# tonyjohnvan/ACE-Step-1.5

Hardware: AMD Instinct MI355X
Metric: seconds/song (240 s audio, 27 DiT steps) (lower is better)
Workload: dtype bf16

## Files before the change

### ace-step-1.5_amd/csrc/gemm.hip

```cpp
#include <hip/hip_ext.h>

#include "kernels.h"
#include "headpost.h"

namespace acehip {
namespace {

constexpr int BK = 64;
constexpr int GROUP_M = 8;

#ifdef GEMM_STAMPS
constexpr int STAMP_WG = 16384;
__device__ unsigned long long g_gemm_stamps[STAMP_WG * 2 * 8];
__device__ __forceinline__ void stamp(int slot, int i, unsigned long long v) {
    if (slot < STAMP_WG * 2) {
        asm volatile("" : "+v"(v));
        g_gemm_stamps[slot * 8 + i] = v;
    }
}
#define GSTAMP(i)                                                                                \
    do {                                                                                         \
        if ((threadIdx.x & 255) == 0 && threadIdx.x < 512) stamp(blockIdx.x * 2 + (threadIdx.x >> 8), i, __builtin_amdgcn_s_memtime()); \
    } while (0)
#define GSTAMP_REAL(i)                                                                           \
    do {                                                                                         \
        if ((threadIdx.x & 255) == 0 && threadIdx.x < 512) stamp(blockIdx.x * 2 + (threadIdx.x >> 8), i, __builtin_amdgcn_s_memrealtime()); \
    } while (0)
#else
#define GSTAMP(i) do {} while (0)
#define GSTAMP_REAL(i) do {} while (0)
#endif

struct ExtEvents {
    hipEvent_t start = nullptr, stop = nullptr;
};
thread_local ExtEvents g_ext_ev;
template <typename... KArgs, typename... Args>
inline void klaunch(void (*kern)(KArgs...), dim3 grid, dim3 block, hipStream_t s, Args... args) {
    if (g_ext_ev.stop) {
        hipEvent_t st = g_ext_ev.start;
        g_ext_ev.start = nullptr;
        hipExtLaunchKernelGGL(kern, grid, block, 0, s, st, g_ext_ev.stop, 0, args...);
    } else {
        kern<<<grid, block, 0, s>>>(args...);
    }
}
__device__ __forceinline__ int swz(int row, int chunk) { return row * 128 + ((chunk ^ ((row >> 1) & 7)) << 4); }

template <int N>
__device__ __forceinline__ void ring_barrier() {
    asm volatile("s_waitcnt vmcnt(%0) lgkmcnt(0)" ::"n"(N) : "memory");
    __builtin_amdgcn_s_barrier();
    asm volatile("" ::: "memory");
}

template <int SM, int SN, int EPI, int CHMAX = 12>
__device__ __forceinline__ void epilogue_tile(const GemmArgs &a, const f32x4 (&acc)[SM][SN], int row0, int col0,
                                              int fr, int fc) {
    static_assert(SN % 2 == 0, "sub-tiles are paired");
    const bool odd = fc & 1;
    const int cpos = (fc >> 1) * 8;
#pragma unroll
    for (int i = 0; i < SM; ++i) {
        const int m = row0 + i * 16 + fr;
        const bool live = m < a.M;
        if constexpr (EPI == EPI_SWIGLU) {
#pragma unroll
            for (int pnl = 0; pnl < SN / 4; ++pnl) {
                f32x4 p0, p1;
                float o[8];
                float g8[8], u8[8];
#pragma unroll
                for (int r = 0; r < 4; ++r) {
                    g8[r] = acc[i][4 * pnl][r];
                    g8[4 + r] = acc[i][4 * pnl + 1][r];
                    u8[r] = acc[i][4 * pnl + 2][r];
                    u8[4 + r] = acc[i][4 * pnl + 3][r];
                }
                rbf_n<8>(g8);
                rbf_n<8>(u8);
#pragma unroll
                for (int r = 0; r < 8; ++r) g8[r] = silu_f(g8[r]);
                rbf_n<8>(g8);
#pragma unroll
                for (int r = 0; r < 4; ++r) {
                    p0[r] = g8[r] * u8[r];
                    p1[r] = g8[4 + r] * u8[4 + r];
                }
                pair8(p0, p1, odd, o);
                const int nout = ((col0 + pnl * 64) >> 1) + (odd ? 16 : 0) + cpos;
                if (live) *(uint4 *)(a.C + (int64_t)m * a.ldc + nout) = pack8(o);
            }
        }
    }
    if constexpr (EPI == EPI_CONV) {
        constexpr int NP = SN / 2;
        uint4 bz[NP];
        float sav[NP][8], sbv[NP][8];
        int colv[NP], phv[NP];
#pragma unroll
        for (int jp = 0; jp < NP; ++jp) {
            const int n = col0 + (2 * jp + (odd ? 1 : 0)) * 16 + cpos;
            phv[jp] = n / a.conv_cout;
            colv[jp] = n - phv[jp] * a.conv_cout;
            bz[jp] = a.bias ? *(const uint4 *)(a.bias + colv[jp]) : make_uint4(0, 0, 0, 0);
            if (a.Cs) {
                const float4 a0 = *(const float4 *)(a.sa + colv[jp]), a1 = *(const float4 *)(a.sa + colv[jp] + 4);
                const float4 b0 = *(const float4 *)(a.sib + colv[jp]), b1 = *(const float4 *)(a.sib + colv[jp] + 4);
                sav[jp][0] = a0.x; sav[jp][1] = a0.y; sav[jp][2] = a0.z; sav[jp][3] = a0.w;
                sav[jp][4] = a1.x; sav[jp][5] = a1.y; sav[jp][6] = a1.z; sav[jp][7] = a1.w;
                sbv[jp][0] = b0.x; sbv[jp][1] = b0.y; sbv[jp][2] = b0.z; sbv[jp][3] = b0.w;
                sbv[jp][4] = b1.x; sbv[jp][5] = b1.y; sbv[jp][6] = b1.z; sbv[jp][7] = b1.w;
            }
        }
// ... 274 lines not shown
        const int r = r0 + RPI * it;
        float x[8], cs[8] = {}, sn[8] = {};
        unpack8(*(const uint4 *)(st + r * PITCH + hh * 128 + d), x);
        if constexpr (MODE >= 2) {
            unpack8(cv[it], cs);
            unpack8(sv[it], sn);
        }
        if constexpr (MODE == 1) head_norm_rope_t<true, false>(x, li, w, cs, sn, h.eps);
        else if constexpr (MODE == 2) head_norm_rope_t<true, true>(x, li, w, cs, sn, h.eps);
        else if constexpr (MODE == 3) head_norm_rope(x, li, norm, w, h.cos != nullptr, cs, sn, h.eps);
        if (m0 + r < a.M) *(uint4 *)(base + (int64_t)bq * bstride + sq * 128) = pack8(x);
        sq += RPI;
        while (sq >= h.S) { sq -= h.S; ++bq; }
    }
}

template <int BM, int NW, int LDS_BYTES, int HPT, typename StoreAcc>
__device__ __forceinline__ void headpost_epilogue(const GemmArgs &a, char *lds, int m0, int n0, int wave, int lane,
                                                  StoreAcc store_acc) {
    static_assert(HPT == 1 || HPT == 2, "one or two heads per tile");
    constexpr int PITCH = 128 * HPT + 8;
    constexpr int RPW = 4 / HPT;
    constexpr int RPI = RPW * NW;
    constexpr int ITER = BM / RPI;
    static_assert(BM % RPI == 0, "rows must split evenly over the iterations");
    static_assert(BM * PITCH * 2 <= LDS_BYTES, "head-post staging tile must fit the operand ring");
    const HeadPostArgs &h = a.hp;
    const int sub = lane >> 4, li = lane & 15, d = li * 8, hh = HPT == 2 ? sub & 1 : 0;
    const int head = (n0 >> 7) + hh;
    const int nqk = h.nq + h.nk;
    const bool norm = head < nqk;
    const bool rope = h.cos != nullptr;
    const int r0 = wave * RPW + (HPT == 2 ? sub >> 1 : sub);
    const int mf = min(m0 + r0, a.M - 1) + h.m_off;
    const int b0 = mf / h.S, s0 = mf - b0 * h.S;
    uint4 cv[ITER], sv[ITER];
    if (rope) {
        int sq = s0;
#pragma unroll
        for (int it = 0; it < ITER; ++it) {
            const int sc = min(sq, h.S - 1);
            cv[it] = *(const uint4 *)(h.cos + (int64_t)sc * 128 + d);
            sv[it] = *(const uint4 *)(h.sin + (int64_t)sc * 128 + d);
            sq += RPI;
            while (sq >= h.S) sq -= h.S;
        }
    }
    bf16_t *base;
    int64_t bstride;
    const int64_t hs = (int64_t)h.S_dst * 128;
    if (head < h.nq) {
        const int64_t hq = h.S_dst_q ? (int64_t)h.S_dst_q * 128 : hs;
        base = h.q + head * hq;
        bstride = h.nq * hq;
    } else if (head < nqk) {
        base = h.k + (head - h.nq) * hs;
        bstride = h.nk * hs;
    } else {
        base = h.v + (head - nqk) * hs;
        bstride = h.nv * hs;
    }
    base += d;
    float w[8] = {};
    if (norm) unpack8(*(const uint4 *)((head < h.nq ? h.qw : h.kw) + d), w);
    bf16_t *st = (bf16_t *)lds;
    __syncthreads();
    store_acc(st, PITCH);
    __syncthreads();
    const bool uniform = HPT == 1 || (h.nq % 2 == 0 && nqk % 2 == 0);
    if (uniform) {
        if ((n0 >> 7) >= nqk)
            headpost_rows<0, ITER, RPI, PITCH>(a, st, m0, r0, hh, li, d, b0, s0, base, bstride, norm, w, cv, sv);
        else if (!rope)
            headpost_rows<1, ITER, RPI, PITCH>(a, st, m0, r0, hh, li, d, b0, s0, base, bstride, norm, w, cv, sv);
        else
            headpost_rows<2, ITER, RPI, PITCH>(a, st, m0, r0, hh, li, d, b0, s0, base, bstride, norm, w, cv, sv);
    } else {
        headpost_rows<3, ITER, RPI, PITCH>(a, st, m0, r0, hh, li, d, b0, s0, base, bstride, norm, w, cv, sv);
    }
}

template <int BM>
constexpr int pp_lds_bytes() { return 2 * (BM + 256) * 128; }
template <int BM, int EPI>
__device__ __forceinline__ void gemm_pp_body(const GemmArgs &a, char *lds, int bid) {
    constexpr int BN = 256, TM = BM / 2, SM = TM / 16, SMH = SM / 2;
    constexpr int ROWS = BM + BN, BUF = ROWS * 128;
    constexpr int NA = BM / 64, NB = BN / 64;
    static_assert(SM % 2 == 0, "A half must be whole 16-row sub-tiles");

    GSTAMP(0);
    GSTAMP_REAL(4);
    const int tid = threadIdx.x, lane = tid & 63, wave = tid >> 6;
    const int wr = wave >> 2, wc = wave & 3;
    const int tilesM = (a.M + BM - 1) / BM, tilesN = a.N / BN;
    const int nwg = tilesM * tilesN;
    const int wg = xcd_remap(bid, nwg);
    const int per_group = GROUP_M * tilesN;
    const int gid = wg / per_group, first_m = gid * GROUP_M;
    const int gsz = min(tilesM - first_m, GROUP_M);
    const int tm = first_m + (wg % per_group) % gsz;
    const int tn = (wg % per_group) / gsz;
    const int m0 = tm * BM, n0 = tn * BN;
#ifdef GEMM_STAMPS
    {
        unsigned xcc;
        asm volatile("s_getreg_b32 %0, hwreg(HW_REG_XCC_ID)" : "=s"(xcc));
        if ((threadIdx.x & 255) == 0) stamp(blockIdx.x * 2 + (threadIdx.x >> 8), 6, ((unsigned long long)wg << 32) | xcc);
    }
#endif

    const bf16_t *srcA[NA], *srcB[NB];
#pragma unroll
    for (int i = 0; i < NA; ++i) {
        const int r = (wave + 8 * i) * 8 + (lane >> 3);
        const int c = (lane & 7) ^ ((r >> 1) & 7);
        srcA[i] = a.A + (int64_t)min(m0 + r, a.M - 1) * a.lda + c * 8;
    }
#pragma unroll
    for (int i = 0; i < NB; ++i) {
        const int r = (wave + 8 * i) * 8 + (lane >> 3);
        const int c = (lane & 7) ^ (((BM + r) >> 1) & 7);
        srcB[i] = a.W + (int64_t)(n0 + r) * a.ldw + c * 8;
    }
    auto stageA = [&](int buf, int k0) {
        char *b = lds + buf * BUF;
        int ko = k0;
        if constexpr (EPI == EPI_CONV) {
            const int cin = a.conv_cin, tap = k0 / cin;
            ko = k0 + tap * (a.conv_dil - 1) * cin + a.conv_a0 * cin;
        }
#pragma unroll
        for (int i = 0; i < NA; ++i) glds16(srcA[i] + ko, b + (wave + 8 * i) * 1024);
    };
    auto stageB = [&](int buf, int k0) {
        char *b = lds + buf * BUF + BM * 128;
#pragma unroll
        for (int i = 0; i < NB; ++i) glds16(srcB[i] + k0, b + (wave + 8 * i) * 1024);
    };
    auto bar = [] {
        __builtin_amdgcn_sched_barrier(0);
        __builtin_amdgcn_s_barrier();
        __builtin_amdgcn_sched_barrier(0);
    };

    f32x4 acc[SM][4];
#pragma unroll
    for (int i = 0; i < SM; ++i)
#pragma unroll
        for (int j = 0; j < 4; ++j) acc[i][j] = f32x4{0.f, 0.f, 0.f, 0.f};

    const int fr = lane & 15, fc = lane >> 4;
    const int arow = wr * TM, brow = BM + wc * 64;

    const int nk = a.K / BK;
    stageB(0, 0);
    stageA(0, 0);
    if (nk > 1) {
        stageB(1, BK);
        asm volatile("s_waitcnt vmcnt(%0)" ::"n"(NB) : "memory");
    } else {
        asm volatile("s_waitcnt vmcnt(0)" ::: "memory");
    }
    bar();
    if (wr == 1) bar();
    GSTAMP(1);

    {
    bf16x8 xa[SMH][2], bf[4][2];
    auto readA = [&](const char *b, int h) {
#pragma unroll
        for (int i = 0; i < SMH; ++i)
#pragma unroll
            for (int ks = 0; ks < 2; ++ks)
                xa[i][ks] = *(const bf16x8 *)(b + swz(arow + (h * SMH + i) * 16 + fr, ks * 4 + fc));
    };
    auto mma = [&](int h) {
        __builtin_amdgcn_sched_barrier(0);
        __builtin_amdgcn_s_setprio(1);
#pragma unroll
        for (int ks = 0; ks < 2; ++ks)
#pragma unroll
            for (int i = 0; i < SMH; ++i)
#pragma unroll
                for (int j = 0; j < 4; ++j)
                    acc[h * SMH + i][j] = __builtin_amdgcn_mfma_f32_16x16x32_bf16(bf[j][ks], xa[i][ks], acc[h * SMH + i][j], 0, 0, 0);
        __builtin_amdgcn_s_setprio(0);
    };
    for (int kt = 0; kt < nk; ++kt) {
        const char *b = lds + (kt & 1) * BUF;
#pragma unroll
        for (int j = 0; j < 4; ++j)
#pragma unroll
            for (int ks = 0; ks < 2; ++ks) bf[j][ks] = *(const bf16x8 *)(b + swz(brow + j * 16 + fr, ks * 4 + fc));
        readA(b, 0);
        if (kt + 1 < nk) stageA((kt + 1) & 1, (kt + 1) * BK);
        asm volatile("s_waitcnt lgkmcnt(0)" ::: "memory");
        bar();
        mma(0);
        bar();
        readA(b, 1);
        if (kt + 2 < nk) {
            stageB(kt & 1, (kt + 2) * BK);
            asm volatile("s_waitcnt vmcnt(%0) lgkmcnt(0)" ::"n"(NB) : "memory");
        } else {
            asm volatile("s_waitcnt vmcnt(0) lgkmcnt(0)" ::: "memory");
        }
        bar();
        mma(1);
        bar();
    }
    }
    if (wr == 0) bar();
    GSTAMP(2);

    if constexpr (EPI == EPI_HEADPOST && BM == 256) {
#pragma unroll
        for (int hf = 0; hf < 2; ++hf)
            headpost_epilogue<128, 8, 2 * BUF, 2>(a, lds, m0 + hf * 128, n0, wave, lane, [&](bf16_t *st, int pitch) {
                if (wr != hf) return;
#pragma unroll
                for (int i = 0; i < SM; ++i)
#pragma unroll
                    for (int j = 0; j < 4; ++j) {
                        float o[4] = {acc[i][j][0], acc[i][j][1], acc[i][j][2], acc[i][j][3]};
                        *(uint2 *)(st + (i * 16 + fr) * pitch + wc * 64 + j * 16 + fc * 4) = pack4(o);
                    }
            });
        return;
    } else if constexpr (EPI == EPI_HEADPOST) {
        headpost_epilogue<BM, 8, 2 * BUF, 2>(a, lds, m0, n0, wave, lane, [&](bf16_t *st, int pitch) {
#pragma unroll
            for (int i = 0; i < SM; ++i)
#pragma unroll
                for (int j = 0; j < 4; ++j) {
                    float o[4] = {acc[i][j][0], acc[i][j][1], acc[i][j][2], acc[i][j][3]};
                    *(uint2 *)(st + (arow + i * 16 + fr) * pitch + wc * 64 + j * 16 + fc * 4) = pack4(o);
                }
        });
        return;
    }

    epilogue_tile<SM, 4, EPI>(a, acc, m0 + arow, n0 + wc * 64, fr, fc);
#ifdef GEMM_STAMPS
    asm volatile("s_waitcnt vmcnt(0)" ::: "memory");
#endif
    GSTAMP(3);
    GSTAMP_REAL(5);
}

template <int BM, int EPI>
__global__ __launch_bounds__(512, 1) void gemm_pp_kernel(GemmArgs a) {
    __shared__ __attribute__((aligned(16))) char lds[pp_lds_bytes<BM>()];
    gemm_pp_body<BM, EPI>(a, lds, blockIdx.x);
}

template <int EPI>
__global__ __launch_bounds__(512, 1) void gemm_pp_split_kernel(GemmArgs a, GemmArgs t, int nmain) {
    __shared__ __attribute__((aligned(16))) char lds[pp_lds_bytes<256>()];
    if ((int)blockIdx.x < nmain) gemm_pp_body<256, EPI>(a, lds, blockIdx.x);
    else gemm_pp_body<128, EPI>(t, lds, blockIdx.x - nmain);
}

template <int BM, int BN, int EPI, int NH = 0>
__global__ __launch_bounds__(256 + 64 * NH, 1) void gemm_w4_kernel(GemmArgs a) {
    constexpr int TM = BM / 2, TN = BN / 2, SM = TM / 16, SN = TN / 16;
    constexpr int ROWS = BM + BN, STAGE = ROWS * 128;
    constexpr int NS = 3 * STAGE <= 160 * 1024 ? 3 : 2;
    constexpr int PW = ROWS / 32;
    static_assert(ROWS % 32 == 0, "staging must split evenly over 4 waves");
    __shared__ __attribute__((aligned(16))) char lds[NS * STAGE];

    GSTAMP(0);
    GSTAMP_REAL(4);
    const int tid = threadIdx.x, lane = tid & 63, wave = tid >> 6;
    const int wm = wave >> 1, wn = wave & 1;
    const int tilesM = (a.M + BM - 1) / BM, tilesN = a.N / BN;
    const int nwg = tilesM * tilesN;
    const int wg = xcd_remap(blockIdx.x, nwg);
    const int per_group = GROUP_M * tilesN;
    const int gid = wg / per_group, first_m = gid * GROUP_M;
    const int gsz = min(tilesM - first_m, GROUP_M);
    const int tm = first_m + (wg % per_group) % gsz;
    const int tn = (wg % per_group) / gsz;
    const int m0 = tm * BM, n0 = tn * BN;
    const int nk = a.K / BK;

    if constexpr (NH > 0) {
        if (__builtin_amdgcn_readfirstlane(wave) >= 4) {
            constexpr int PPH = 4 * PW / NH;
            static_assert((4 * PW) % NH == 0 && (NS - 1) * PPH < 64, "helper pieces / vmcnt field");
            const int h = wave - 4;
            const bf16_t *hs[PPH];
#pragma unroll
            for (int i = 0; i < PPH; ++i) {
                const int q = h + NH * i, r = q * 8 + (lane >> 3);
                const int c = (lane & 7) ^ ((r >> 1) & 7);
                if (r < BM) hs[i] = a.A + (int64_t)min(m0 + r, a.M - 1) * a.lda + c * 8;
                else hs[i] = a.W + (int64_t)(n0 + r - BM) * a.ldw + c * 8;
            }
            auto fill = [&](int buf, int k0) {
#pragma unroll
                for (int i = 0; i < PPH; ++i) glds16(hs[i] + k0, lds + buf * STAGE + (h + NH * i) * 1024);
            };
            for (int t = 0; t < NS; ++t) fill(t, min(t, nk - 1) * BK);
            asm volatile("s_waitcnt vmcnt(%0)" ::"n"((NS - 1) * PPH) : "memory");
            __builtin_amdgcn_s_barrier();
            for (int kt = 0; kt < nk; ++kt) {
                asm volatile("s_waitcnt vmcnt(%0)" ::"n"((NS - 2) * PPH) : "memory");
                __builtin_amdgcn_s_barrier();
                asm volatile("" ::: "memory");
                fill(kt % NS, min(kt + NS, nk - 1) * BK);
            }
            asm volatile("s_waitcnt vmcnt(0)" ::: "memory");
            if constexpr (EPI == EPI_HEADPOST) {
                __syncthreads();
                __syncthreads();
            }
            return;
        }
    }

    const bf16_t *src[PW];
#pragma unroll
    for (int i = 0; i < PW; ++i) {
        const int r = (wave + 4 * i) * 8 + (lane >> 3);
        const int c = (lane & 7) ^ ((r >> 1) & 7);
        if (r < BM) src[i] = a.A + (int64_t)min(m0 + r, a.M - 1) * a.lda + c * 8;
        else src[i] = a.W + (int64_t)(n0 + r - BM) * a.ldw + c * 8;
    }
    auto stage1 = [&](int buf, int k0, int i) { glds16(src[i] + k0, lds + buf * STAGE + (wave + 4 * i) * 1024); };
// ... 116 lines not shown
        case EPI_SWIGLU: klaunch(gemm_pp_kernel<BM, EPI_SWIGLU>, dim3(tiles), dim3(512), s, a); break;
        case EPI_CONV:
            if constexpr (BM == 256 || BM == 128) {
                gemm_pp_kernel<BM, EPI_CONV><<<tiles, 512, 0, s>>>(a);
                break;
            }
            return fail(-1, "gemm: the conv epilogue runs on the 256- or 128-row ping-pong tile");
        case EPI_HEADPOST:
            if constexpr (BM == 256 || BM == 192 || BM == 128) {
                gemm_pp_kernel<BM, EPI_HEADPOST><<<tiles, 512, 0, s>>>(a);
                break;
            }
            return fail(-1, "gemm: head-post epilogue needs the 256-, 192- or 128-row ping-pong tile");
        default: return fail(-1, "gemm: bad epilogue");
    }
    HIP_TRY(hipGetLastError());
    return 0;
}

template <int BM, int BN, int WM, int WN, int STAGES, int NH = 0>
int launch(const GemmArgs &a, hipStream_t s) {
    if (a.N % BN) return fail(-1, "gemm: N not a multiple of the tile");
    const int tiles = ((a.M + BM - 1) / BM) * (a.N / BN);
    constexpr int NT = WM * WN * 64 + 64 * NH;
    switch (a.epi) {
        case EPI_STORE: gemm_kernel<BM, BN, WM, WN, STAGES, EPI_STORE, NH><<<tiles, NT, 0, s>>>(a); break;
        case EPI_GATED_RES: gemm_kernel<BM, BN, WM, WN, STAGES, EPI_GATED_RES, NH><<<tiles, NT, 0, s>>>(a); break;
        case EPI_RES: gemm_kernel<BM, BN, WM, WN, STAGES, EPI_RES, NH><<<tiles, NT, 0, s>>>(a); break;
        case EPI_SWIGLU: klaunch(gemm_kernel<BM, BN, WM, WN, STAGES, EPI_SWIGLU, NH>, dim3(tiles), dim3(NT), s, a); break;
        default: return fail(-1, "gemm: bad epilogue for this variant");
    }
    HIP_TRY(hipGetLastError());
    return 0;
}

}

int gemm_variant(const GemmArgs &a, int variant, hipStream_t s) {
    switch (variant) {
        case 0: return launch<128, 128, 2, 2, 2>(a, s);
        case 7: return launch_pp<256>(a, s);
        case 8: return launch_pp<192>(a, s);
        case 9: return launch_pp<128>(a, s);
        case 13: return knobs().gemm_helpers ? launch_w4<192, 128, 2>(a, s) : launch_w4<192, 128>(a, s);
        case 16: return launch<128, 64, 4, 1, 4>(a, s);
        case 17: return launch<128, 64, 4, 1, 4, 2>(a, s);
        default: return fail(-1, "gemm: bad variant (0, 7, 8, 9, 13, 16, 17)");
    }
}

#ifdef GEMM_STAMPS
}
extern "C" int acehip_diag_gemm_stamps(void *host, int n_wg) {
    n_wg = std::min(n_wg, acehip::STAMP_WG);
    HIP_TRY(hipMemcpyFromSymbol(host, HIP_SYMBOL(acehip::g_gemm_stamps), (size_t)n_wg * 2 * 8 * 8));
    return 0;
}
extern "C" int acehip_diag_gemm_stamps_clear(void) {
    void *p = nullptr;
    HIP_TRY(hipGetSymbolAddress(&p, HIP_SYMBOL(acehip::g_gemm_stamps)));
    HIP_TRY(hipMemset(p, 0, sizeof(acehip::g_gemm_stamps)));
    return 0;
}
namespace acehip {
#endif

bool gemm_ext_events(hipEvent_t start, hipEvent_t stop) {
    const bool consumed = g_ext_ev.stop && !g_ext_ev.start;
    g_ext_ev.start = start;
    g_ext_ev.stop = stop;
    return consumed;
}

static int num_cus() {
    static int n = 0;
    if (!n) {
        int dev = 0;
        if (hipGetDevice(&dev) != hipSuccess ||
            hipDeviceGetAttribute(&n, hipDeviceAttributeMultiprocessorCount, dev) != hipSuccess || n <= 0)
            n = 256;
    }
    return n;
}

static bool use_w4s(int64_t M, int N) {
    if (N % 128) return false;
    const int cus = num_cus();
    const int64_t t = ((M + 191) / 192) * (N / 128);
    return t <= cus && t * 4 >= (int64_t)cus * 3;
}

int gemm_pick_variant(int64_t M, int N) {
    if (use_w4s(M, N) && (N % 256 || ((M + 191) / 192) * (N / 256) <= num_cus() / 2)) return 13;
    if (N % 256) return 0;
    const int cus = num_cus();
    const int64_t t7 = ((M + 255) / 256) * (N / 256), t8 = ((M + 191) / 192) * (N / 256);
    if (t8 <= cus / 2) return 0;
    const int64_t t9 = ((M + 127) / 128) * (N / 256);
    if (t8 <= cus && t9 <= cus) return 9;
    const double c7 = (double)((t7 + cus - 1) / cus) * 1.093, c8 = (double)((t8 + cus - 1) / cus);
    return c7 < c8 ? 7 : 8;
}

static int splitk_finish(const GemmArgs &a, const GemmArgs &p, int splits, hipStream_t s);

static int splitk_bn(const GemmArgs &) {
    const int f = knobs().splitk_bn;
    if (f) return f == 64 ? 64 : 128;
    return 64;
}
static void fill_defer(const GemmArgs &a, int splits, RowAdd *defer);
static int gemm_splitk(const GemmArgs &a, int splits, hipStream_t s, RowAdd *defer = nullptr) {
    GemmArgs p = a;
    const int nk = a.K / BK;
    p.kper = (nk + splits - 1) / splits;
    splits = (nk + p.kper - 1) / p.kper;
    const int bn = splitk_bn(a);
    const int tiles = ((a.M + 127) / 128) * (a.N / bn);
    if (bn == 64) gemm_kernel<128, 64, 4, 1, 3, EPI_PARTIAL><<<dim3(tiles, splits), 256, 0, s>>>(p);
    else if (a.N <= 4096) gemm_kernel<128, 128, 2, 2, 3, EPI_PARTIAL><<<dim3(tiles, splits), 256, 0, s>>>(p);
    else gemm_kernel<128, 128, 2, 2, 2, EPI_PARTIAL><<<dim3(tiles, splits), 256, 0, s>>>(p);
    HIP_TRY(hipGetLastError());
    if (defer) {
        fill_defer(a, splits, defer);
        return 0;
    }
    return splitk_finish(a, p, splits, s);
}

static void fill_defer(const GemmArgs &a, int splits, RowAdd *defer) {
    defer->xw = a.C;
    defer->part = (const float *)a.ws;
    defer->splits = splits;
    defer->prows = a.M;
    defer->plane = (int64_t)a.M * a.N;
    defer->gate = a.epi == EPI_GATED_RES ? a.gate : nullptr;
    defer->gate_bstride = a.gate_bstride;
    defer->gate_rpb = a.epi == EPI_GATED_RES ? a.rows_per_batch : 1;
}

static int splitk_finish(const GemmArgs &a, const GemmArgs &p, int splits, hipStream_t s) {
    if (a.epi == EPI_HEADPOST && knobs().splitk_fuse) {
        HeadPostArgs h = a.hp;
        h.part = (const float *)a.ws;
        h.splits = splits;
        h.plane = (int64_t)a.M * a.N;
        h.ld_src = a.N;
        return head_post(h, s);
    }
    bf16_t *out = a.C;
    int64_t ldo = a.ldc;
    if (a.epi == EPI_HEADPOST) {
        out = (bf16_t *)((char *)a.ws + (size_t)splits * a.M * a.N * 4);
        ldo = a.N;
    }
    const int nout = a.epi == EPI_SWIGLU ? a.N / 2 : a.N;
    const int64_t thr = (int64_t)a.M * nout / 4;
    splitk_epilogue_kernel<<<(unsigned)((thr + 255) / 256), 256, 0, s>>>(p, splits, out, ldo);
    HIP_TRY(hipGetLastError());
    if (a.epi == EPI_HEADPOST) {
        HeadPostArgs h = a.hp;
        h.src = out;
        h.ld_src = a.N;
        return head_post(h, s);
    }
    return 0;
}

static int gemm_tail_split(const GemmArgs &a, int v, hipStream_t s) {
    if (a.epi != EPI_SWIGLU && a.epi != EPI_STORE && a.epi != EPI_HEADPOST) return 1;
    if (!knobs().gemm_tailsplit) return 1;
    const int BMv = v == 7 ? 256 : 192, cus = num_cus();
    const int64_t nN = a.N / 256, tiles = (int64_t)((a.M + BMv - 1) / BMv) * nN;
    const int64_t full = tiles / cus, rem = tiles - full * cus;
    if (full < 1 || rem == 0 || rem * 5 > (int64_t)cus * 3) return 1;
    const int64_t M1 = (full * cus / nN) * BMv;
    if (M1 <= 0 || M1 >= a.M) return 1;
    if (((a.M - M1 + 127) / 128) * (a.N / 128) > 2 * (int64_t)cus) return 1;
    GemmArgs hd = a;
    hd.M = (int)M1;
    GemmArgs tl = a;
    tl.M = a.M - (int)M1;
    tl.A = a.A + M1 * a.lda;
    if (a.epi == EPI_HEADPOST) tl.hp.m_off += (int)M1;
    else tl.C = a.C + M1 * a.ldc;
    const bool pp128 = a.N % 256 == 0 && ((tl.M + 127) / 128) * nN <= cus;
    if (a.epi == EPI_HEADPOST && !pp128) return 1;
    if (pp128 && v == 7) {
        const int nmain = (int)(full * cus / nN * nN), ntail = ((tl.M + 127) / 128) * (int)nN;
        if (nmain % 8 == 0 && nmain == (hd.M / 256) * (int)nN && hd.M % 256 == 0) {
            if (a.epi == EPI_SWIGLU) klaunch(gemm_pp_split_kernel<EPI_SWIGLU>, dim3(nmain + ntail), dim3(512), s, hd, tl, nmain);
            else if (a.epi == EPI_HEADPOST) gemm_pp_split_kernel<EPI_HEADPOST><<<nmain + ntail, 512, 0, s>>>(hd, tl, nmain);
            else gemm_pp_split_kernel<EPI_STORE><<<nmain + ntail, 512, 0, s>>>(hd, tl, nmain);
            HIP_TRY(hipGetLastError());
            return 0;
        }
    }
    int rc = gemm_variant(hd, v, s);
    if (rc) return rc;
    return gemm_variant(tl, pp128 ? 9 : 0, s);
}

static int launch_conv64(const GemmArgs &a, hipStream_t s) {
    const int tiles = ((a.M + 63) / 64) * (a.N / 256);
    gemm_pp_kernel<64, EPI_CONV><<<tiles, 512, 0, s>>>(a);
    HIP_TRY(hipGetLastError());
    return 0;
}

int gemm_conv(const GemmArgs &a, hipStream_t s) {
    if (a.epi != EPI_CONV || (!a.C && !a.Cs) || (a.Cs && (!a.sa || !a.sib)) || a.conv_cin <= 0 || a.conv_dil < 1 ||
        a.conv_ostride < 1 || a.conv_cout <= 0 || a.conv_cout % 8 || a.N % a.conv_cout || a.conv_lout <= 0 || a.M <= 0)
        return fail(-1, "gemm_conv: EPI_CONV with an output, snake parameters and conv geometry required");
    if (a.N % 256 || a.conv_cin % BK || a.K % a.conv_cin || a.lda != a.conv_cin || a.ldw != a.K || a.ldc != a.conv_cout)
        return fail(-1, "gemm_conv: N % 256, cin % 64, K = taps·cin and dense layouts required");
    if (a.res && (a.N != a.conv_cout || a.ldr != a.N || a.conv_ostride != 1 || a.conv_ooff != 0 || a.conv_lout != a.M))
        return fail(-1, "gemm_conv: a residual needs one phase with output row = m");
    if ((int64_t)((a.M + 255) / 256) * (a.N / 256) >= (1ll << 31)) return fail(-1, "gemm_conv: grid too large");
    const int64_t t256 = (int64_t)((a.M + 255) / 256) * (a.N / 256);
    if (t256 * 4 <= num_cus()) return launch_conv64(a, s);
    if (t256 * 2 <= num_cus()) return launch_pp<128>(a, s);
    return launch_pp<256>(a, s);
}

int gemm(const GemmArgs &a, hipStream_t s, RowAdd *defer) {
    if (defer) defer->part = nullptr;
    if (a.M <= 0) return 0;
    if (a.N % 128 || a.K % BK || a.K <= 0)
        return fail(-1, "gemm: N%128 / K%64 violated (M=" + std::to_string(a.M) + " N=" +
                            std::to_string(a.N) + " K=" + std::to_string(a.K) + ")");
    if ((a.lda | a.ldw | a.ldc) % 8) return fail(-1, "gemm: leading dims must be multiples of 8");
    if (a.epi == EPI_GATED_RES && (!a.gate || a.rows_per_batch <= 0)) return fail(-1, "gemm: gate");
    if ((a.epi == EPI_GATED_RES || a.epi == EPI_RES) && !a.res) return fail(-1, "gemm: res");
    if (a.epi == EPI_HEADPOST) {
        const HeadPostArgs &h = a.hp;
        if (a.N % 256 || h.S <= 0 || (int64_t)h.B * h.S != a.M || (h.nq + h.nk + h.nv) * 128 != a.N ||
            h.S_dst < h.S || (h.S_dst_q && h.S_dst_q < h.S) || (h.nq && !h.qw) || (h.nk && !h.kw) || (h.cos == nullptr) != (h.sin == nullptr))
            return fail(-1, "gemm: head-post arguments inconsistent with the GEMM shape");
    }
    const Knobs &kn = knobs();
    const bool dfr = defer && kn.splitk_fuse && (a.epi == EPI_GATED_RES || a.epi == EPI_RES) && a.res == a.C &&
                     a.ldr == a.ldc && a.ldc == a.N;
    if (a.epi == EPI_SWIGLU && a.M <= 128 && a.N % 64 == 0 && kn.smallm_wholek) return gemm_variant(a, kn.smallm_wholek == 2 ? 17 : 16, s);
    if (a.ws && a.N % 128 == 0 && a.K % BK == 0 && (a.N % 256 == 0 || a.epi != EPI_HEADPOST)) {
        const int cus = num_cus();
        const int64_t tiles = ((a.M + 127) / 128) * (a.N / 128);
        const int nk = a.K / BK;
        if (tiles * 2 <= cus && nk >= 8) {
            const int64_t tb = ((a.M + 127) / 128) * (a.N / splitk_bn(a));
            int splits = (int)std::min<int64_t>(std::min<int64_t>(16, nk / 4), (cus + tb - 1) / tb);
            const size_t need = (size_t)splits * a.M * a.N * 4 + (size_t)a.M * a.N * 2;
            if (splits >= 2 && need <= a.ws_bytes) return gemm_splitk(a, splits, s, dfr ? defer : nullptr);
        }
    }
    if (a.epi == EPI_HEADPOST) {
        const int64_t t192 = (int64_t)((a.M + 191) / 192) * (a.N / 256);
        const bool small = t192 * 2 <= num_cus();
        if (small && use_w4s(a.M, a.N)) return gemm_variant(a, 13, s);
        if (small && a.ws && (size_t)a.M * a.N * 2 <= a.ws_bytes) {
            GemmArgs st = a;
            st.epi = EPI_STORE;
            st.bias = nullptr;
            st.C = (bf16_t *)a.ws;
            st.ldc = a.N;
            int rc = gemm_variant(st, 0, s);
            if (rc) return rc;
            HeadPostArgs hh = a.hp;
            hh.src = st.C;
            hh.ld_src = a.N;
            return head_post(hh, s);
        }
        if (kn.gemm_hp_tail && a.N % 256 == 0) {
            const int cus = num_cus();
            const int64_t nN = a.N / 256, t7 = ((a.M + 255) / 256) * nN, t8 = ((a.M + 191) / 192) * nN;
            const double c_split = (double)(t7 / cus) * 1.093 + 0.6, c8 = (double)((t8 + cus - 1) / cus);
            if (t7 >= cus && c_split < c8) {
                const int rc = gemm_tail_split(a, 7, s);
                if (rc <= 0) return rc;
            }
        }
        return gemm_variant(a, 8, s);
    }
    const int v = gemm_pick_variant(a.M, a.N);
    if (v == 7 || v == 8) {
        const int rc = gemm_tail_split(a, v, s);
        if (rc <= 0) return rc;
    }
    return gemm_variant(a, v, s);
}

}
```

### ace-step-1.5_amd/csrc/kernels.h

```cpp
#pragma once
#include "common.h"

namespace acehip {

struct Knobs {
    int gemm_tailsplit = 1;
    int gemm_helpers = 1;
    int splitk_fuse = 1;
    int splitk_bn = 0;
    int smallm_wholek = 2;
    int attn_pw = 2;
    int attn_persist = 1;
    int attn_small = 1;
    int attn_small_mask = 1;
    int attn_small_causal = 1;
    int attn_cus = 0;
    int attn_streamk = 1;
    int fuse_rowadd = 1;
    int dit_dedup = 1;
    int dit_graph = 0;
    int gemm_hp_tail = 1;
    int convt = 1;
    int conv7 = 2;
    int convp = 3;
    int ru7 = 2;
    int vae_snake_in = 1;
    int kv_group_kib = 262144;
    unsigned gen = 0;
};
const Knobs &knobs();

struct HeadPostArgs {
    const bf16_t *src; int64_t ld_src;
    int B, S;
    int nq, nk, nv;
    const bf16_t *qw, *kw;
    const bf16_t *cos, *sin;
    bf16_t *q, *k, *v;
    int S_dst;
    float eps;
    const float *part = nullptr; int splits = 0; int64_t plane = 0;
    int m_off = 0;
    int S_dst_q = 0;
};
enum GemmEpi {
    EPI_STORE = 0,
    EPI_GATED_RES = 1,
    EPI_RES = 2,
    EPI_SWIGLU = 3,
    EPI_HEADPOST = 4,
};


struct GemmArgs {
    const bf16_t *A; int64_t lda;
    const bf16_t *W; int64_t ldw;
    bf16_t *C; int64_t ldc;
    int M, N, K;
    int epi;
    const bf16_t *bias;
    const bf16_t *res; int64_t ldr;
    const bf16_t *gate; int64_t gate_bstride; int rows_per_batch;
    HeadPostArgs hp;
    void *ws; size_t ws_bytes;
    int kper;
    const float *sa, *sib;
    bf16_t *Cs;
    int conv_cin, conv_dil, conv_a0, conv_ostride, conv_ooff, conv_cout;
    int64_t conv_lout;
};
constexpr int EPI_PARTIAL = 5;
constexpr int EPI_CONV = 6;
constexpr size_t GEMM_WS_BYTES = (size_t)48 << 20;
struct RowAdd;
int gemm(const GemmArgs &a, hipStream_t s, RowAdd *defer = nullptr);
int gemm_variant(const GemmArgs &a, int variant, hipStream_t s);
int gemm_conv(const GemmArgs &a, hipStream_t s);
bool gemm_ext_events(hipEvent_t start, hipEvent_t stop);

int gemv_small(const bf16_t *x, int64_t ldx, const bf16_t *W, const bf16_t *bias, bf16_t *y,
               int64_t ldy, int M, int N, int K, int act, hipStream_t s, bf16_t *act_scratch = nullptr);
int bcast_rows(const bf16_t *src, int64_t n, bf16_t *dst, int rows, hipStream_t s);
int timestep_sinusoid(const float *t, const float *t_r, int t_stride, int use_diff, int Bc,
                      const float *freqs, bf16_t *emb, hipStream_t s);
int add_bf16(const bf16_t *a, const bf16_t *b, bf16_t *out, int64_t n, hipStream_t s);
int modulation(const bf16_t *tables, int n_tables, int rows, const bf16_t *proj, int Bc, int D,
               bf16_t *mod, hipStream_t s);
int pack_patches(const bf16_t *xt, const bf16_t *ctx, int Bx, int Bc, int T, int S, bf16_t *X,
                 hipStream_t s);
int gather_head_row(const bf16_t *V, int KV, int Le, int H, bf16_t *out, hipStream_t s);
int add_row_bcast(bf16_t *X, const bf16_t *c, int rows, int D, hipStream_t s);
int copy_cols(const bf16_t *src, int64_t lds, bf16_t *dst, int64_t ldd, int M, int C, hipStream_t s);
int crop_rows(const bf16_t *src, int Bc, int rows_src, int rows_dst, int C, bf16_t *dst,
              hipStream_t s);

struct RowAdd {
    bf16_t *xw = nullptr;
    const bf16_t *v = nullptr;
    int from = 0;
    const float *part = nullptr;
    int splits = 0, prows = 0;
    int64_t plane = 0;
    const bf16_t *gate = nullptr;
// ... 90 lines not shown
```

### ace-step-1.5_amd/csrc/knobs.hip

```cpp
#include <atomic>
#include <cstdlib>
#include <mutex>

#include "kernels.h"
#include "../../include/acehip.h"

namespace acehip {
namespace {

int env_int(const char *name, int dflt) {
    const char *e = getenv(name);
    return (e && *e) ? atoi(e) : dflt;
}

Knobs read_env() {
    Knobs k;
    k.gemm_tailsplit = env_int("ACEHIP_GEMM_TAILSPLIT", 1);
    k.gemm_helpers = env_int("ACEHIP_GEMM_HELPERS", 1);
    k.splitk_fuse = env_int("ACEHIP_SPLITK_FUSE", 1);
    k.splitk_bn = env_int("ACEHIP_SPLITK_BN", 0);
    k.smallm_wholek = env_int("ACEHIP_SMALLM_WHOLEK", 2);
    k.attn_pw = env_int("ACEHIP_ATTN_PW", 2);
    k.attn_persist = env_int("ACEHIP_ATTN_PERSIST", 1);
    k.attn_small = env_int("ACEHIP_ATTN_SMALL", 1);
    k.attn_small_mask = env_int("ACEHIP_ATTN_SMALL_MASK", 1);
    k.attn_small_causal = env_int("ACEHIP_ATTN_SMALL_CAUSAL", 1);
    k.attn_cus = env_int("ACEHIP_ATTN_CUS", 0);
    k.attn_streamk = env_int("ACEHIP_ATTN_STREAMK", 1);
    k.fuse_rowadd = env_int("ACEHIP_FUSE_ROWADD", 1);
    k.dit_dedup = env_int("ACEHIP_DIT_DEDUP", 1);
    k.dit_graph = env_int("ACEHIP_DIT_GRAPH", 0);
    k.conv7 = env_int("ACEHIP_CONV7", 2);
    k.convt = env_int("ACEHIP_CONVT", 1);
    k.gemm_hp_tail = env_int("ACEHIP_GEMM_HPTAIL", 1);
    k.convp = env_int("ACEHIP_CONVP", 3);
    k.ru7 = env_int("ACEHIP_RU7", 2);
    k.kv_group_kib = env_int("ACEHIP_KV_GROUP_KIB", 262144);
    k.vae_snake_in = env_int("ACEHIP_VAE_SNAKE_IN", 1);
    if (k.kv_group_kib <= 0) k.kv_group_kib = 262144;
    return k;
}

std::mutex g_mu;
Knobs g_knobs;
std::atomic<bool> g_loaded{false};

}

const Knobs &knobs() {
    if (!g_loaded.load(std::memory_order_acquire)) {
        std::lock_guard<std::mutex> lk(g_mu);
        if (!g_loaded.load(std::memory_order_relaxed)) {
            g_knobs = read_env();
            g_loaded.store(true, std::memory_order_release);
        }
    }
    return g_knobs;
}

}

extern "C" int acehip_reload_knobs(void) {
    std::lock_guard<std::mutex> lk(acehip::g_mu);
    const unsigned gen = acehip::g_knobs.gen + 1;
    acehip::g_knobs = acehip::read_env();
    acehip::g_knobs.gen = gen;
    acehip::g_loaded.store(true, std::memory_order_release);
    return 0;
}
```

Before: 0.5004.

## Add persistent SwiGLU GEMM kernel overlapping next tile prologue with epilogue

Adds a persistent ping-pong GEMM kernel for the SwiGLU epilogue. Each workgroup walks several 256-row tiles and then 128-row tail tiles, issuing the next tile's global-to-LDS prologue loads before running the current tile's store epilogue. The goal is to hide per-tile launch and prologue latency and to replace the separate tail-split launch. It also adds scalar-base-plus-offset LDS DMA addressing and a CU-count cap knob. The trade-off is more complex vmcnt bookkeeping that depends on a fixed epilogue store count.

```diff
diff --git a/ace-step-1.5_amd/csrc/gemm.hip b/ace-step-1.5_amd/csrc/gemm.hip
--- a/ace-step-1.5_amd/csrc/gemm.hip
+++ b/ace-step-1.5_amd/csrc/gemm.hip
@@ -18,18 +18,20 @@
         g_gemm_stamps[slot * 8 + i] = v;
     }
 }
-#define GSTAMP(i)                                                                                \
+#define GSTAMP_AT(slot, i)                                                                       \
     do {                                                                                         \
-        if ((threadIdx.x & 255) == 0 && threadIdx.x < 512) stamp(blockIdx.x * 2 + (threadIdx.x >> 8), i, __builtin_amdgcn_s_memtime()); \
+        if ((threadIdx.x & 255) == 0 && threadIdx.x < 512) stamp((slot) * 2 + (threadIdx.x >> 8), i, __builtin_amdgcn_s_memtime()); \
     } while (0)
-#define GSTAMP_REAL(i)                                                                           \
+#define GSTAMP_REAL_AT(slot, i)                                                                  \
     do {                                                                                         \
-        if ((threadIdx.x & 255) == 0 && threadIdx.x < 512) stamp(blockIdx.x * 2 + (threadIdx.x >> 8), i, __builtin_amdgcn_s_memrealtime()); \
+        if ((threadIdx.x & 255) == 0 && threadIdx.x < 512) stamp((slot) * 2 + (threadIdx.x >> 8), i, __builtin_amdgcn_s_memrealtime()); \
     } while (0)
 #else
-#define GSTAMP(i) do {} while (0)
-#define GSTAMP_REAL(i) do {} while (0)
+#define GSTAMP_AT(slot, i) do {} while (0)
+#define GSTAMP_REAL_AT(slot, i) do {} while (0)
 #endif
+#define GSTAMP(i) GSTAMP_AT(blockIdx.x, i)
+#define GSTAMP_REAL(i) GSTAMP_REAL_AT(blockIdx.x, i)
 
 struct ExtEvents {
     hipEvent_t start = nullptr, stop = nullptr;
@@ -470,17 +472,9 @@
 
 template <int BM>
 constexpr int pp_lds_bytes() { return 2 * (BM + 256) * 128; }
-template <int BM, int EPI>
-__device__ __forceinline__ void gemm_pp_body(const GemmArgs &a, char *lds, int bid) {
-    constexpr int BN = 256, TM = BM / 2, SM = TM / 16, SMH = SM / 2;
-    constexpr int ROWS = BM + BN, BUF = ROWS * 128;
-    constexpr int NA = BM / 64, NB = BN / 64;
-    static_assert(SM % 2 == 0, "A half must be whole 16-row sub-tiles");
-
-    GSTAMP(0);
-    GSTAMP_REAL(4);
-    const int tid = threadIdx.x, lane = tid & 63, wave = tid >> 6;
-    const int wr = wave >> 2, wc = wave & 3;
+template <int BM>
+__device__ __forceinline__ void pp_tile_origin(const GemmArgs &a, int bid, int slot, int &m0, int &n0) {
+    constexpr int BN = 256;
     const int tilesM = (a.M + BM - 1) / BM, tilesN = a.N / BN;
     const int nwg = tilesM * tilesN;
     const int wg = xcd_remap(bid, nwg);
@@ -489,50 +483,118 @@
     const int gsz = min(tilesM - first_m, GROUP_M);
     const int tm = first_m + (wg % per_group) % gsz;
     const int tn = (wg % per_group) / gsz;
-    const int m0 = tm * BM, n0 = tn * BN;
+    m0 = tm * BM;
+    n0 = tn * BN;
 #ifdef GEMM_STAMPS
     {
         unsigned xcc;
         asm volatile("s_getreg_b32 %0, hwreg(HW_REG_XCC_ID)" : "=s"(xcc));
-        if ((threadIdx.x & 255) == 0) stamp(blockIdx.x * 2 + (threadIdx.x >> 8), 6, ((unsigned long long)wg << 32) | xcc);
+        if ((threadIdx.x & 255) == 0) {
+            stamp(slot * 2 + (threadIdx.x >> 8), 6, ((unsigned long long)wg << 32) | xcc);
+            stamp(slot * 2 + (threadIdx.x >> 8), 7, blockIdx.x);
+        }
     }
 #endif
-
-    const bf16_t *srcA[NA], *srcB[NB];
-#pragma unroll
-    for (int i = 0; i < NA; ++i) {
-        const int r = (wave + 8 * i) * 8 + (lane >> 3);
-        const int c = (lane & 7) ^ ((r >> 1) & 7);
-        srcA[i] = a.A + (int64_t)min(m0 + r, a.M - 1) * a.lda + c * 8;
-    }
-#pragma unroll
-    for (int i = 0; i < NB; ++i) {
-        const int r = (wave + 8 * i) * 8 + (lane >> 3);
-        const int c = (lane & 7) ^ (((BM + r) >> 1) & 7);
-        srcB[i] = a.W + (int64_t)(n0 + r) * a.ldw + c * 8;
-    }
-    auto stageA = [&](int buf, int k0) {
-        char *b = lds + buf * BUF;
-        int ko = k0;
-        if constexpr (EPI == EPI_CONV) {
-            const int cin = a.conv_cin, tap = k0 / cin;
-            ko = k0 + tap * (a.conv_dil - 1) * cin + a.conv_a0 * cin;
-        }
-#pragma unroll
-        for (int i = 0; i < NA; ++i) glds16(srcA[i] + ko, b + (wave + 8 * i) * 1024);
-    };
-    auto stageB = [&](int buf, int k0) {
-        char *b = lds + buf * BUF + BM * 128;
-#pragma unroll
-        for (int i = 0; i < NB; ++i) glds16(srcB[i] + k0, b + (wave + 8 * i) * 1024);
-    };
-    auto bar = [] {
-        __builtin_amdgcn_sched_barrier(0);
-        __builtin_amdgcn_s_barrier();
-        __builtin_amdgcn_sched_barrier(0);
-    };
-
-    f32x4 acc[SM][4];
+}
+
+template <int BM>
+struct PPSrcPtr {
+    static constexpr int NA = BM / 64, NB = 4;
+    const bf16_t *pa[NA], *pb[NB];
+    __device__ __forceinline__ void set(const GemmArgs &a, int m0, int n0, int wave, int lane) {
+#pragma unroll
+        for (int i = 0; i < NA; ++i) {
+            const int r = (wave + 8 * i) * 8 + (lane >> 3);
+            const int c = (lane & 7) ^ ((r >> 1) & 7);
+            pa[i] = a.A + (int64_t)min(m0 + r, a.M - 1) * a.lda + c * 8;
+        }
+#pragma unroll
+        for (int i = 0; i < NB; ++i) {
+            const int r = (wave + 8 * i) * 8 + (lane >> 3);
+            const int c = (lane & 7) ^ (((BM + r) >> 1) & 7);
+            pb[i] = a.W + (int64_t)(n0 + r) * a.ldw + c * 8;
+        }
+    }
+    __device__ __forceinline__ void dmaA(int i, int k0, char *dst) const { glds16(pa[i] + k0, dst); }
+    __device__ __forceinline__ void dmaB(int i, int k0, char *dst) const { glds16(pb[i] + k0, dst); }
+};
+
+__device__ __forceinline__ void glds16_s(const char *sbase, uint32_t voff, char *lds_dst) {
+    const uint32_t la = (uint32_t)(uintptr_t)(const __attribute__((address_space(3))) char *)lds_dst;
+    asm volatile("s_mov_b32 m0, %0\n\ts_nop 0\n\tglobal_load_lds_dwordx4 %1, %2" ::"s"(la), "v"(voff), "s"(sbase)
+                 : "memory");
+}
+
+template <int BM>
+struct PPSrcOff {
+    static constexpr int NA = BM / 64, NB = 4;
+    const char *ba, *bb;
+    uint32_t oa[NA], ob, bstep;
+    __device__ __forceinline__ void set(const GemmArgs &a, int m0, int n0, int wave, int lane) {
+        ba = (const char *)(a.A + (int64_t)m0 * a.lda);
+        bb = (const char *)(a.W + (int64_t)n0 * a.ldw);
+        bstep = 64u * (uint32_t)a.ldw * 2u;
+        const int r0 = wave * 8 + (lane >> 3);
+        const uint32_t c16 = (uint32_t)((lane & 7) ^ ((r0 >> 1) & 7)) * 16u;
+        ob = (uint32_t)r0 * (uint32_t)a.ldw * 2u + c16;
+        const int last = a.M - 1 - m0;
+#pragma unroll
+        for (int i = 0; i < NA; ++i) oa[i] = (uint32_t)min(r0 + 64 * i, last) * (uint32_t)a.lda * 2u + c16;
+    }
+    __device__ __forceinline__ void dmaA(int i, int k0, char *dst) const { glds16_s(ba + (int64_t)k0 * 2, oa[i], dst); }
+    __device__ __forceinline__ void dmaB(int i, int k0, char *dst) const {
+        glds16_s(bb + (uint64_t)i * bstep + (int64_t)k0 * 2, ob, dst);
+    }
+};
+
+template <int BM, int EPI, typename Src>
+__device__ __forceinline__ void pp_stageA(const GemmArgs &a, char *lds, const Src &src, int wave, int buf, int k0) {
+    constexpr int BUF = (BM + 256) * 128;
+    char *b = lds + buf * BUF;
+    int ko = k0;
+    if constexpr (EPI == EPI_CONV) {
+        const int cin = a.conv_cin, tap = k0 / cin;
+        ko = k0 + tap * (a.conv_dil - 1) * cin + a.conv_a0 * cin;
+    }
+#pragma unroll
+    for (int i = 0; i < Src::NA; ++i) src.dmaA(i, ko, b + (wave + 8 * i) * 1024);
+}
+template <int BM, typename Src>
+__device__ __forceinline__ void pp_stageB(char *lds, const Src &src, int wave, int buf, int k0) {
+    constexpr int BUF = (BM + 256) * 128;
+    char *b = lds + buf * BUF + BM * 128;
+#pragma unroll
+    for (int i = 0; i < Src::NB; ++i) src.dmaB(i, k0, b + (wave + 8 * i) * 1024);
+}
+__device__ __forceinline__ void pp_bar() {
+    __builtin_amdgcn_sched_barrier(0);
+    __builtin_amdgcn_s_barrier();
+    __builtin_amdgcn_sched_barrier(0);
+}
+template <int BM, int EPI, typename Src>
+__device__ __forceinline__ void pp_prologue_issue(const GemmArgs &a, char *lds, const Src &src, int wave) {
+    pp_stageB<BM>(lds, src, wave, 0, 0);
+    pp_stageA<BM, EPI>(a, lds, src, wave, 0, 0);
+    if (a.K > BK) pp_stageB<BM>(lds, src, wave, 1, BK);
+}
+
+constexpr int PP_SWIGLU_STORES = 256 / 2 / 16;
+
+template <int BM, int EPI, bool PERSIST, typename Src>
+__device__ __forceinline__ void pp_main(const GemmArgs &a, char *lds, const Src &src, f32x4 (&acc)[BM / 32][4],
+                                        int slot, int pend) {
+    constexpr int BN = 256, TM = BM / 2, SM = TM / 16, SMH = SM / 2;
+    constexpr int ROWS = BM + BN, BUF = ROWS * 128;
+    constexpr int NB = BN / 64;
+    static_assert(SM % 2 == 0, "A half must be whole 16-row sub-tiles");
+    const int tid = threadIdx.x, lane = tid & 63;
+    int wave = tid >> 6;
+    if constexpr (PERSIST) wave = __builtin_amdgcn_readfirstlane(wave);
+    const int wr = wave >> 2, wc = wave & 3;
+    auto stageA = [&](int buf, int k0) { pp_stageA<BM, EPI>(a, lds, src, wave, buf, k0); };
+    auto stageB = [&](int buf, int k0) { pp_stageB<BM>(lds, src, wave, buf, k0); };
+    auto bar = [] { pp_bar(); };
+
 #pragma unroll
     for (int i = 0; i < SM; ++i)
 #pragma unroll
@@ -542,17 +604,29 @@
     const int arow = wr * TM, brow = BM + wc * 64;
 
     const int nk = a.K / BK;
-    stageB(0, 0);
-    stageA(0, 0);
-    if (nk > 1) {
-        stageB(1, BK);
-        asm volatile("s_waitcnt vmcnt(%0)" ::"n"(NB) : "memory");
+    if constexpr (!PERSIST) {
+        stageB(0, 0);
+        stageA(0, 0);
+        if (nk > 1) {
+            stageB(1, BK);
+            asm volatile("s_waitcnt vmcnt(%0)" ::"n"(NB) : "memory");
+        } else {
+            asm volatile("s_waitcnt vmcnt(0)" ::: "memory");
+        }
     } else {
-        asm volatile("s_waitcnt vmcnt(0)" ::: "memory");
+        if (pend < 0) pp_prologue_issue<BM, EPI>(a, lds, src, wave);
+        __builtin_amdgcn_sched_barrier(0);
+        if (pend > 0) {
+            if (nk > 1) asm volatile("s_waitcnt vmcnt(%0)" ::"n"(NB + PP_SWIGLU_STORES) : "memory");
+            else asm volatile("s_waitcnt vmcnt(%0)" ::"n"(PP_SWIGLU_STORES) : "memory");
+        } else {
+            if (nk > 1) asm volatile("s_waitcnt vmcnt(%0)" ::"n"(NB) : "memory");
+            else asm volatile("s_waitcnt vmcnt(0)" ::: "memory");
+        }
     }
     bar();
     if (wr == 1) bar();
-    GSTAMP(1);
+    GSTAMP_AT(slot, 1);
 
     {
     bf16x8 xa[SMH][2], bf[4][2];
@@ -600,8 +674,16 @@
     }
     }
     if (wr == 0) bar();
-    GSTAMP(2);
-
+    GSTAMP_AT(slot, 2);
+}
+
+template <int BM, int EPI>
+__device__ __forceinline__ void pp_epilogue(const GemmArgs &a, char *lds, const f32x4 (&acc)[BM / 32][4], int m0, int n0) {
+    constexpr int TM = BM / 2, SM = TM / 16, BUF = (BM + 256) * 128;
+    const int tid = threadIdx.x, lane = tid & 63, wave = tid >> 6;
+    const int wr = wave >> 2, wc = wave & 3;
+    const int fr = lane & 15, fc = lane >> 4;
+    const int arow = wr * TM;
     if constexpr (EPI == EPI_HEADPOST && BM == 256) {
 #pragma unroll
         for (int hf = 0; hf < 2; ++hf)
@@ -630,11 +712,88 @@
     }
 
     epilogue_tile<SM, 4, EPI>(a, acc, m0 + arow, n0 + wc * 64, fr, fc);
+}
+
+template <int BM, int EPI>
+__device__ __forceinline__ void gemm_pp_body(const GemmArgs &a, char *lds, int bid) {
+    GSTAMP(0);
+    GSTAMP_REAL(4);
+    const int tid = threadIdx.x, lane = tid & 63, wave = tid >> 6;
+    int m0, n0;
+    pp_tile_origin<BM>(a, bid, blockIdx.x, m0, n0);
+    PPSrcPtr<BM> src;
+    src.set(a, m0, n0, wave, lane);
+    f32x4 acc[BM / 32][4];
+    pp_main<BM, EPI, false>(a, lds, src, acc, blockIdx.x, -1);
+    pp_epilogue<BM, EPI>(a, lds, acc, m0, n0);
+    if constexpr (EPI == EPI_HEADPOST) return;
 #ifdef GEMM_STAMPS
     asm volatile("s_waitcnt vmcnt(0)" ::: "memory");
 #endif
     GSTAMP(3);
     GSTAMP_REAL(5);
+}
+
+template <int EPI>
+__global__ __launch_bounds__(512, 1) void gemm_pp_persist_kernel(GemmArgs a, GemmArgs t, int nmain, int ntot) {
+    static_assert(EPI == EPI_SWIGLU, "the early prologue needs an epilogue that leaves LDS alone and a known store count");
+    __shared__ __attribute__((aligned(16))) char lds[pp_lds_bytes<256>()];
+    const int tid = threadIdx.x, lane = tid & 63, wave = __builtin_amdgcn_readfirstlane(tid >> 6);
+    const int G = gridDim.x;
+    int i = blockIdx.x;
+    int pend = -1;
+    int m0 = 0, n0 = 0;
+    GSTAMP_AT(i, 0);
+    GSTAMP_REAL_AT(i, 4);
+    PPSrcOff<256> src;
+    PPSrcOff<128> tsrc;
+    if (i < nmain) {
+        pp_tile_origin<256>(a, i, i, m0, n0);
+        src.set(a, m0, n0, wave, lane);
+    }
+    for (; i < nmain; i += G) {
+        f32x4 acc[8][4];
+        pp_main<256, EPI, true>(a, lds, src, acc, i, pend);
+        const int cm0 = m0, cn0 = n0, nx = i + G;
+        pend = cm0 + 256 <= a.M ? 1 : 0;
+        if (nx < ntot) {
+            GSTAMP_AT(nx, 0);
+            GSTAMP_REAL_AT(nx, 4);
+        }
+        if (nx < nmain) {
+            pp_tile_origin<256>(a, nx, nx, m0, n0);
+            src.set(a, m0, n0, wave, lane);
+            pp_prologue_issue<256, EPI>(a, lds, src, wave);
+        } else if (nx < ntot) {
+            pp_tile_origin<128>(t, nx - nmain, nx, m0, n0);
+            tsrc.set(t, m0, n0, wave, lane);
+            pp_prologue_issue<128, EPI>(t, lds, tsrc, wave);
+        }
+        __builtin_amdgcn_sched_barrier(0);
+        pp_epilogue<256, EPI>(a, lds, acc, cm0, cn0);
+        __builtin_amdgcn_sched_barrier(0);
+        GSTAMP_AT(i, 3);
+        GSTAMP_REAL_AT(i, 5);
+    }
+    for (; i < ntot; i += G) {
+        if (pend < 0) {
+            pp_tile_origin<128>(t, i - nmain, i, m0, n0);
+            tsrc.set(t, m0, n0, wave, lane);
+        }
+        f32x4 acc[4][4];
+        pp_main<128, EPI, true>(t, lds, tsrc, acc, i, pend);
+        pend = -1;
+        pp_epilogue<128, EPI>(t, lds, acc, m0, n0);
+#ifdef GEMM_STAMPS
+        asm volatile("s_waitcnt vmcnt(0)" ::: "memory");
+#endif
+        GSTAMP_AT(i, 3);
+        GSTAMP_REAL_AT(i, 5);
+        if (i + G < ntot) {
+            GSTAMP_AT(i + G, 0);
+            GSTAMP_REAL_AT(i + G, 4);
+        }
+    }
 }
 
 template <int BM, int EPI>
@@ -917,6 +1076,18 @@
     }
     return n;
 }
+static int plan_cus() {
+    const int cap = knobs().gemm_cus, n = num_cus();
+    return cap > 0 && cap < n ? cap : n;
+}
+
+static int launch_pp_persist(const GemmArgs &hd, const GemmArgs &tl, int nmain, int ntail, hipStream_t s) {
+    const int grid = std::min(plan_cus(), nmain + ntail);
+    if (ntail > grid) return fail(-1, "gemm: persistent walk with more tail tiles than workgroups");
+    klaunch(gemm_pp_persist_kernel<EPI_SWIGLU>, dim3(grid), dim3(512), s, hd, tl, nmain, nmain + ntail);
+    HIP_TRY(hipGetLastError());
+    return 0;
+}
 
 static bool use_w4s(int64_t M, int N) {
     if (N % 128) return false;
@@ -928,7 +1099,7 @@
 int gemm_pick_variant(int64_t M, int N) {
     if (use_w4s(M, N) && (N % 256 || ((M + 191) / 192) * (N / 256) <= num_cus() / 2)) return 13;
     if (N % 256) return 0;
-    const int cus = num_cus();
+    const int cus = plan_cus();
     const int64_t t7 = ((M + 255) / 256) * (N / 256), t8 = ((M + 191) / 192) * (N / 256);
     if (t8 <= cus / 2) return 0;
     const int64_t t9 = ((M + 127) / 128) * (N / 256);
@@ -1005,7 +1176,7 @@
 static int gemm_tail_split(const GemmArgs &a, int v, hipStream_t s) {
     if (a.epi != EPI_SWIGLU && a.epi != EPI_STORE && a.epi != EPI_HEADPOST) return 1;
     if (!knobs().gemm_tailsplit) return 1;
-    const int BMv = v == 7 ? 256 : 192, cus = num_cus();
+    const int BMv = v == 7 ? 256 : 192, cus = plan_cus();
     const int64_t nN = a.N / 256, tiles = (int64_t)((a.M + BMv - 1) / BMv) * nN;
     const int64_t full = tiles / cus, rem = tiles - full * cus;
     if (full < 1 || rem == 0 || rem * 5 > (int64_t)cus * 3) return 1;
@@ -1023,6 +1194,8 @@
     if (a.epi == EPI_HEADPOST && !pp128) return 1;
     if (pp128 && v == 7) {
         const int nmain = (int)(full * cus / nN * nN), ntail = ((tl.M + 127) / 128) * (int)nN;
+        if (a.epi == EPI_SWIGLU && knobs().gemm_persist && nmain == (hd.M / 256) * (int)nN && hd.M % 256 == 0)
+            return launch_pp_persist(hd, tl, nmain, ntail, s);
         if (nmain % 8 == 0 && nmain == (hd.M / 256) * (int)nN && hd.M % 256 == 0) {
             if (a.epi == EPI_SWIGLU) klaunch(gemm_pp_split_kernel<EPI_SWIGLU>, dim3(nmain + ntail), dim3(512), s, hd, tl, nmain);
             else if (a.epi == EPI_HEADPOST) gemm_pp_split_kernel<EPI_HEADPOST><<<nmain + ntail, 512, 0, s>>>(hd, tl, nmain);
@@ -1121,6 +1294,10 @@
         const int rc = gemm_tail_split(a, v, s);
         if (rc <= 0) return rc;
     }
+    if (v == 7 && a.epi == EPI_SWIGLU && knobs().gemm_persist) {
+        const int64_t tiles = (int64_t)((a.M + 255) / 256) * (a.N / 256);
+        if (tiles > plan_cus() && tiles < (1ll << 30)) return launch_pp_persist(a, a, (int)tiles, 0, s);
+    }
     return gemm_variant(a, v, s);
 }
 
diff --git a/ace-step-1.5_amd/csrc/kernels.h b/ace-step-1.5_amd/csrc/kernels.h
--- a/ace-step-1.5_amd/csrc/kernels.h
+++ b/ace-step-1.5_amd/csrc/kernels.h
@@ -19,6 +19,8 @@
     int fuse_rowadd = 1;
     int dit_dedup = 1;
     int dit_graph = 0;
+    int gemm_persist = 1;
+    int gemm_cus = 0;
     int gemm_hp_tail = 1;
     int convt = 1;
     int conv7 = 2;
diff --git a/ace-step-1.5_amd/csrc/knobs.hip b/ace-step-1.5_amd/csrc/knobs.hip
--- a/ace-step-1.5_amd/csrc/knobs.hip
+++ b/ace-step-1.5_amd/csrc/knobs.hip
@@ -33,6 +33,8 @@
     k.conv7 = env_int("ACEHIP_CONV7", 2);
     k.convt = env_int("ACEHIP_CONVT", 1);
     k.gemm_hp_tail = env_int("ACEHIP_GEMM_HPTAIL", 1);
+    k.gemm_persist = env_int("ACEHIP_GEMM_PERSIST", 1);
+    k.gemm_cus = env_int("ACEHIP_GEMM_CUS", 0);
     k.convp = env_int("ACEHIP_CONVP", 3);
     k.ru7 = env_int("ACEHIP_RU7", 2);
     k.kv_group_kib = env_int("ACEHIP_KV_GROUP_KIB", 262144);
```

New measurement: 0.4954 (median of 6 runs). 1.0% less time.
